# refresh-bio/fqsqueezer

Measured on AMD Instinct MI355X. Metric: Mbases/s compressed (DNA stream, SE sorted), higher is better.
Workload: dtype u64; 1 GPU; 1000000x150bp SE, G=7500000 (seed 2+rank), -om s -gs 8 -qm n -im n; workers_T=64, blocks=256, per_gpu=one independent file per GPU

## Files before the change

### fqsqueezer_amd/codec.py

```python
from __future__ import annotations

import ctypes as C
import os
from typing import List, Optional

import numpy as np

_PKG = os.path.dirname(os.path.abspath(__file__))
DEFAULT_LIB = os.path.join(_PKG, "libfqsx.so")

STAT_NAMES = ["gprobe", "gslot", "lprobe", "lslot", "gins", "gins_slot", "siv_words", "ctx_slots",
              "coded", "lins", "mail", "bases", "siv_saved", "dec_refetch"]


class FqsxError(RuntimeError):
    pass


_P, _INT, _U32, _U64, _HDR = C.c_void_p, C.c_int, C.c_uint32, C.c_uint64, C.c_char_p
_OUT, _U64S, _MS, _IN = C.POINTER(C.c_void_p), C.POINTER(C.c_uint64), C.POINTER(C.c_double), C.POINTER(C.c_char_p)
_ID_ENCODE = [_P, _P, _P, _U32, _INT, _OUT, _U64S]
_ID_DECODE = [_P, _IN, _P, _U32, _INT, _OUT, _OUT]

_ABI = {
    "fqsx_dna_create": (_INT, [_HDR, _INT, _OUT]),
    "fqsx_dna_create_on_partition": (_INT, [_HDR, _INT, _U32, _U32, _OUT]),
    "fqsx_dna_destroy": (None, [_P]),
    "fqsx_dna_use_chunked_tables": (_INT, [_P]),
    "fqsx_dna_encode_block": (_INT, [_P, _P, _P, _U32, _U32, _OUT, _U64S]),
    "fqsx_dna_encode_block_dev": (_INT, [_P, _P, _P, _P, _U32, _U32, _OUT, _U64S]),
    "fqsx_dna_decode_block": (_INT, [_P, _IN, _P, _P, _U32, _U32, _P]),
    "fqsx_dna_decode_block_dev": (_INT, [_P, _IN, _P, _P, _U32, _U32, _OUT]),
    "fqsx_dna_stats": (_INT, [_P, _U64S]),
    "fqsx_dna_capacity": (_INT, [_P, _U64S]),
    "fqsx_dna_set_profiling": (_INT, [_P, _INT]),
    "fqsx_dna_kernel_times": (_INT, [_P, _MS]),
    "fqsx_qual_create": (_INT, [_HDR, _INT, _OUT]),
    "fqsx_qual_destroy": (None, [_P]),
    "fqsx_qual_encode_block": (_INT, [_P, _P, _P, _U32, _OUT, _U64S]),
    "fqsx_qual_encode_block_dev": (_INT, [_P, _P, _P, _P, _U32, _OUT, _U64S]),
    "fqsx_qual_decode_block": (_INT, [_P, _IN, _P, _P, _U32, _P]),
    "fqsx_qual_decode_block_dev": (_INT, [_P, _IN, _P, _P, _U32, _OUT]),
    "fqsx_qual_contexts": (_INT, [_P, _P]),
    "fqsx_qual_set_profiling": (_INT, [_P, _INT]),
    "fqsx_qual_kernel_times": (_INT, [_P, _MS]),
# ... 637 lines not shown
```

### fqsqueezer_amd/csrc/fqsx_api.hip

```cpp
#include "fqsx_kernels.h"
#include "fqsx_qual.h"
#include "fqsx_qdec.h"
#include "../../include/fqsx.h"
#include "fqsx_vm.h"
#include "fqsx_rt.h"
#include <sys/resource.h>

#ifndef FQSX_EMU
#include <dlfcn.h>
#include <rccl/rccl.h>
#endif
#include <algorithm>
#include <cstdio>
#include <cstdlib>
#include <cstring>
#include <string>
#include <vector>

extern "C" const char *fqsx_last_error(void) { return g_err.c_str(); }
extern "C" const char *fqsx_version(void) {
#ifdef FQSX_EMU
  return "fqsx 0.1 (host emulation build - tests only)";
#else
  return "fqsx 0.1 (HIP gfx950)";
// ... 24 lines not shown
  }
  insert_phase_body(cfg, &sm, FQ_BLOCK / 3, FQ_BLOCK % 3);
  if (cfg.sys_scope) fq_release_system();
}
FQ_KERNEL64 void k_compact_generic(const u8 *out, u64 out_cap, const u64 *lens, u8 *dst) {
  const u32 tid = FQ_BLOCK;
  u64 off = 0;
  for (u32 t = 0; t < tid; ++t) off += lens[t];
  const u64 n = lens[tid] <= out_cap ? lens[tid] : 0;
  const u8 *src = out + (u64)tid * out_cap;
  for (u64 i = FQ_LANE; i < n; i += FQ_WAVE) dst[off + i] = src[i];
}
FQ_KERNEL64 void k_clear_local(DevCfg cfg, u64 nb_slots, u64 ns_slots) {
  if (phase_skip(cfg)) return;
  const u64 stride = (u64)FQ_NBLOCKS * FQ_WAVE, first = (u64)FQ_BLOCK * FQ_WAVE + FQ_LANE;
  for (u64 i = first; i < nb_slots; i += stride) cfg.l_b.slots[i] = 0;
  for (u64 i = first; i < ns_slots; i += stride) cfg.l_s.slots[i] = 0;
  for (u64 i = first; i < 2ull * cfg.T; i += stride) cfg.l_s.filled[i] = 0;
}
FQ_KERNEL64 void k_finish_block(DevCfg cfg, u64 *lens , u64 *end ) {
  if (FQ_LANE == 0) {
    if (FQ_BLOCK == 0) { end[2 * cfg.T] = cfg.err[0]; end[2 * cfg.T + 1] = cfg.err[1]; }
    if (cfg.err[1]) return;
    finish_block_body(cfg, FQ_BLOCK);
    lens[FQ_BLOCK] = cfg.ws[FQ_BLOCK].out_len;
    end[FQ_BLOCK] = cfg.ws[FQ_BLOCK].out_len;
    end[cfg.T + FQ_BLOCK] = cfg.ctx_filled[FQ_BLOCK];
  }
}
FQ_KERNEL64 void k_gather_stats(DevCfg cfg, u64 *out) {
  for (u32 i = FQ_LANE; i < 64; i += FQ_WAVE) {
    u64 s = 0;
    for (u32 t = 0; t < cfg.T; ++t) s += cfg.ws[t].stat[i];
    out[i] = s;
  }
}
FQ_DEV void part_split(const DevCfg &cfg, u32 &kind, u32 &blk) {
  kind = 0;
  blk = FQ_BLOCK;
  for (; kind < 2; ++kind) {
    const u32 g = cfg.T * cfg.mail[kind].n_tiles;
    if (blk < g) break;
    blk -= g;
  }
}
FQ_KERNEL64 void k_part_count(DevCfg cfg) {
  FQ_SHARED u32 hist[256];
  u32 kind, blk;
  if (phase_skip(cfg)) return;
  part_split(cfg, kind, blk);
  part_count_body(cfg, kind, blk, hist);
}
FQ_KERNEL64 void k_part_scan(DevCfg cfg) {
  if (phase_skip(cfg)) return;
  part_scan_body(cfg, FQ_BLOCK / cfg.T, FQ_BLOCK % cfg.T);
}
FQ_DEV void part_dstoff_leader(const DevCfg &cfg, u32 kind, u32 *demand , u32 seg1);
FQ_KERNEL64 void k_part_dstoff(DevCfg cfg, u32 *demand , u32 seg1) {
  if (cfg.err[0] || (cfg.err[1] && cfg.err[1] != seg1)) {
    if (FQ_BLOCK == 0 && FQ_LANE == 0) demand[2 * cfg.T] = cfg.err[0];
    return;
  }
  part_dstoff_leader(cfg, FQ_BLOCK, demand, seg1);
}
FQ_DEV void part_dstoff_leader(const DevCfg &cfg, u32 kind, u32 *demand, u32 seg1) {
  part_dstoff_body(cfg, kind);
  if (kind != MAIL_P)
// ... 1097 lines not shown
  if ((rc = dalloc(c, &p, T * sizeof(u32), true))) return rc;
  cfg.ctx_filled = (u32 *)p;
  {
    std::vector<u16> tpl(SM_OFF_BYTE, 0);
    auto fill = [&](u32 off, u32 entries, u32 stride, u32 n) {
      for (u32 e = 0; e < entries; ++e) {
        for (u32 i = 0; i < n; ++i) tpl[off + e * stride + i] = 1;
        tpl[off + e * stride + n] = (u16)n;
      }
    };
    fill(SM_OFF_FLAGS, 256, SM_FLAGS_N + 1, SM_FLAGS_N);
    fill(SM_OFF_NS, 32, SM_NS_N + 1, SM_NS_N);
    fill(SM_OFF_PSF, 65536, SM_PSF_N + 1, SM_PSF_N);
    fill(SM_OFF_PSNB, 65536, 6, cfg.ps_nobytes_n);
    fill(SM_OFF_NIB, 68, SM_NIB_N + 1, SM_NIB_N);
    tpl.resize(SM_TOTAL_U16, 0);
    fill(SM_OFF_MID, 1, SM_NIB_N + 1, SM_NIB_N);
    if ((rc = dalloc(c, &p, (u64)T * SM_TOTAL_U16 * sizeof(u16), false))) return rc;
    cfg.small = (u16 *)p;
    if ((rc = h2d(c, cfg.small, tpl.data(), tpl.size() * sizeof(u16)))) return rc;
    DEVCHK(dev_sync(c));
    for (u32 t = 1; t < T; ++t)
      if ((rc = d2d(c, cfg.small + (u64)t * SM_TOTAL_U16, cfg.small, tpl.size() * sizeof(u16)))) return rc;
    if ((rc = dalloc(c, &p, (u64)T * SM_LAZY_ENTRIES, true))) return rc;
    cfg.byte_init = (u8 *)p;
  }
  {
    std::vector<WState> ws(1);
    memset(ws.data(), 0, sizeof(WState));
    for (int g = 0; g < 4; ++g) {
      mt_seed(ws[0].mt[g], 5481);
      ws[0].mt_idx[g] = 624;
    }
    if ((rc = dalloc(c, &p, (u64)T * sizeof(WState), false))) return rc;
    cfg.ws = (WState *)p;
    for (u32 t = 0; t < T; ++t)
      if ((rc = h2d(c, cfg.ws + t, ws.data(), sizeof(WState)))) return rc;
    DEVCHK(dev_sync(c));
  }
  for (u32 k = 0; k < 3; ++k) {
    if ((rc = dalloc(c, &p, (u64)T * sizeof(u32), true))) return rc;
    cfg.mail[k].n = (u32 *)p;
    if ((rc = dalloc(c, &p, (u64)T * sizeof(u32), true))) return rc;
    cfg.mail[k].dst_tot = (u32 *)p;
    if ((rc = dalloc(c, &p, ((u64)T + 1) * sizeof(u32), true))) return rc;
    cfg.mail[k].dst_off = (u32 *)p;
    if ((rc = mail_alloc(c, k, FQSX_TILE))) return rc;
  }
  c->paired = cfg.mode >= 2;
  c->gpe_cap = c->lpe_cap = 0;
  if (c->paired) {
    c->gpe_cap = pow2_at_least(std::max<u64>(1024, (1ull << 20) / T));
    if (const char *e = getenv("FQSX_PTAB_INIT")) c->gpe_cap = pow2_at_least(std::max<u64>(64, strtoull(e, nullptr, 10)));
    if ((rc = ptab_alloc(c, cfg.g_pe, T, c->gpe_cap, true))) return rc;
    c->lpe_cap = 1024;
    if ((rc = ptab_alloc(c, cfg.l_pe, T, c->lpe_cap, true))) return rc;
    if ((rc = dalloc(c, &p, (u64)T * sizeof(u32), true))) return rc;
    cfg.pe_n = (u32 *)p;
    if ((rc = dalloc(c, &p, (3 * (u64)T + 1) * sizeof(u32), true))) return rc;
    cfg.pe_bkt_n = (u32 *)p;
    cfg.pe_bkt_cur = cfg.pe_bkt_n + 2 * T + 1;
  }
  {
    u8 ident[256];
    for (u32 i = 0; i < 256; ++i) ident[i] = (u8)i;
    if ((rc = dalloc(c, &p, 256, false))) return rc;
    c->d_vmap = (u8 *)p;
// ... 1952 lines not shown
```

### fqsqueezer_amd/csrc/fqsx_dev.h

```cpp
#pragma once
#include "fqsx_layout.h"
#include "fqsx_rc.h"

#define FQSX_RR 6u
#define FQSX_SW 4u
#define FQSX_NSC 3u
#define FQSX_SCR FQSX_NSC
#define FQSX_RQ 256u
struct SpecBuf {
  u32 h_read, h_i0, h_n;
  u32 h_epoch;
  u32 h_pub;
  u32 h_fix_lane, h_fix_end;
  u32 h_pq_lo[2];
  u32 h_np, h_nlp;
  u64 h_ns, h_nls;
  u64 sp_sdir[6][FQSX_SPEC];
  u64 sp_src[6][FQSX_SPEC];
  u8 sp_scur[6][FQSX_SPEC];
  u64 sp_key[10][FQSX_SPEC];
  u8 sp_kind[FQSX_SPEC];
  u64 sp_cq[FQSX_SPEC];
  u8 sp_lvz[FQSX_SPEC];
  u8 sp_flag[FQSX_SPEC];
// ... 144 lines not shown
  u32 pe_n;
  const u8 *din;
  u64 din_len, din_pos;
  RcDec dec;
  u32 la[3];
  u32 pq_lo[2];
  bool lqh;
  u32 lq_pub[2];
  u8 *rdp;
  SpecBuf *sb;
  bool scout;
  bool sc_abandoned;
  u32 sc_read;
  u32 sc_epoch;
  bool sc_poll;
  u32 nsc;
  bool sc_reqmode;
  const u8 *rq_p;
  u32 rq_size;
  bool rq_rev;
  u32 sc_taken;
  u32 sc_base;
  bool rq_early;
  bool rq_noscout;
  HeadRec *rec;
  u32 rec_idx;
  bool piped;
  u32 cq_tail, cq_head;
  bool rcq;
  u32 rq_tail;
  u64 c_r_sym;
  u64 st[ST_N];
  u64 tm[FQSX_TM_SLOTS];
  u32 err;
};
#define FQSX_TRACE_LAUNCHES 4096u
#define FQSX_TRACE_W 32u
#ifdef FQSX_TIMING
#define TM_STAMP(cfg, tid, launch, slot) do { if ((cfg).trace && (launch) < FQSX_TRACE_LAUNCHES && FQ_LANE == 0) (cfg).trace[((u64)(launch) * (cfg).T + (tid)) * FQSX_TRACE_W + (slot)] = fq_clock(); } while (0)
#define TM_TRACE_VAL(cfg, tid, launch, slot, v) do { if ((cfg).trace && (launch) < FQSX_TRACE_LAUNCHES && FQ_LANE == 0) (cfg).trace[((u64)(launch) * (cfg).T + (tid)) * FQSX_TRACE_W + (slot)] = (v); } while (0)
#else
#define TM_STAMP(cfg, tid, launch, slot) ((void)0)
#define TM_TRACE_VAL(cfg, tid, launch, slot, v) ((void)0)
#endif
#ifdef FQSX_TIMING
#define TM_BEGIN(v) u64 v = fq_clock()
#define TM_END(w, slot, v) (w).tm[slot] += fq_clock() - (v)
#define TM_COUNT(w, slot) (w).tm[slot] += 1
#if defined(FQSX_TIMING_PE)
#define TM_END_SP(w, slot, v) ((void)0)
#define TM_END_MD(w, slot, v) ((void)0)
#define TM_END_PE(w, slot, v) TM_END(w, slot, v)
#elif defined(FQSX_TIMING_MODELS)
#define TM_END_SP(w, slot, v) ((void)0)
#define TM_END_MD(w, slot, v) TM_END(w, slot, v)
#else
#define TM_END_SP(w, slot, v) TM_END(w, slot, v)
#define TM_END_MD(w, slot, v) ((void)0)
#endif
#ifndef TM_END_PE
#define TM_END_PE(w, slot, v) ((void)0)
#endif
#else
#define TM_BEGIN(v) ((void)0)
#define TM_END(w, slot, v) ((void)0)
#define TM_COUNT(w, slot) ((void)0)
// ... 2469 lines not shown
#endif
  TM_END(w, TM_CR_RC, t_rc);
  return L;
}
FQ_DEV u32 cq_process(Wk &w, u32 head, u32 avail) {
  u32 L = code_run(w, head, avail < 64 ? avail : 64);
  if (L == 0) {
    code_one(w, head);
    TM_COUNT(w, CN_P2);
    L = 1;
  }
  return L;
}
FQ_DEV void code_chunk(Wk &w, const u8 *p, u32 size, u32 i0, u32 j0, u32 m, bool reversed, u32 hist_start, bool &first) {
  if (m <= j0) return;
  TM_BEGIN(t_c2);
  WgShared *sm = w.sm;
  code_keys(w, p, size, i0, j0, m, reversed, hist_start);
  TM_END(w, TM_KEYS, t_c2);
  TM_BEGIN(t_cq);
  if (!cq_wait_space(w, m - j0)) return;
  for (u32 j = j0 + FQ_LANE; j < m; j += FQ_WAVE) {
    const u32 e = (w.cq_tail + (j - j0)) & (FQSX_CQ - 1);
    const u32 kind = w.sb->sp_kind[j];
    const u32 nk = kind == SK_LETTER ? 10u : 7u;
    for (u32 l = 0; l < nk; ++l) sm->cq_key[l][e] = w.sb->sp_key[l][j];
    sm->cq_kind[e] = (u8)(kind | (first && j == j0 ? SK_RESET : 0u));
    sm->cq_rsym[e] = w.sb->sp_rsym[j];
  }
  FQ_SYNC();
  first = false;
  cq_publish(w, m - j0);
  TM_END(w, TX_CHUNKQ, t_cq);
  if (!w.piped) {
    while (w.cq_head != w.cq_tail && !w.err) w.cq_head += cq_process(w, w.cq_head, w.cq_tail - w.cq_head);
    TM_END(w, TM_FAST, t_c2);
  }
}

#if FQ_WAVE > 1
FQ_DEV u32 grp_hash(u64 g) { return (u32)((g * 0x9E3779B97F4A7C15ull) >> 52); }
FQ_DEV void qm_set(u32 *bits, u64 g) {
  const u64 h = g * 0x9E3779B97F4A7C15ull;
  const u32 a = (u32)(h >> 51), b = (u32)(h >> 38) & 8191u;
  atomicOr(&bits[a >> 5], 1u << (a & 31));
  atomicOr(&bits[b >> 5], 1u << (b & 31));
}
FQ_DEV bool qm_test(const u32 *bits, u64 g) {
  const u64 h = g * 0x9E3779B97F4A7C15ull;
  const u32 a = (u32)(h >> 51), b = (u32)(h >> 38) & 8191u;
  return ((bits[a >> 5] >> (a & 31)) & (bits[b >> 5] >> (b & 31)) & 1u) != 0;
}
struct ConfMasks { u64 quiet, ncb, ncs; };
FQ_DEV ConfMasks conflict_masks(Wk &w, u32 n, bool want_quiet) {
  ConfMasks R;
  R.quiet = R.ncb = R.ncs = 0;
  SpecBuf *sb = w.sb;
  WgShared *sm = w.sm;
  const DevCfg *cfg = w.cfg;
  const u32 lane = FQ_LANE;
  FQ_SYNC();
  const u32 xfl = lane < n && sb->sp_flag[lane] == 3 ? sb->sx_flag[lane] : 0u;
  const bool cand = (xfl & SX_VALID) != 0, qcand = (xfl & (SX_VALID | SX_HITS)) == SX_VALID;
  const u64 A = wave_ballot(cand);
  if (popc64(A) < 4) return R;
  const u32 lo_b = w.pq_lo[0], hi_b = w.mn[MAIL_B], lo_s = w.pq_lo[1], hi_s = w.mn[MAIL_S];
// ... 639 lines not shown
      sm->cq_kind[e] = SK_RAW;
      sm->cq_rsym[e] = 5;
    }
    FQ_SYNC();
    cq_publish(w, n_raw);
  }
  if (!same) {
    mail_push(w, MAIL_P, rec->pmail[0]);
    mail_push(w, MAIL_P, rec->pmail[1]);
    w.pm.dir = rec->kdir[0]; w.pm.rc = rec->krc[0]; w.pm.cur = rec->kcur[0];
    w.sm_.dir = rec->kdir[1]; w.sm_.rc = rec->krc[1]; w.sm_.cur = rec->kcur[1];
    w.bm.dir = rec->kdir[2]; w.bm.rc = rec->krc[2]; w.bm.cur = rec->kcur[2];
    w.pm_u = w.pm; w.sm_u = w.sm_; w.bm_u = w.bm;
    w.cor_pos = 0;
    w.N_run = rec->n_run;
    w.rdp = sm->rd[idx % FQSX_HD];
    w.sc_read = idx;
    w.sc_abandoned = false;
    u32 hist[4] = {rec->hist[0], rec->hist[1], rec->hist[2], rec->hist[3]};
    TM_END(w, TM_READ_HEAD, t_head);
    suffix(w, p, size, false);
    add_s_letters(w, hist);
    w.st[ST_BASES] += size;
    if (w.sc_abandoned && has_next) scout_restart(w, idx + 1, w.cfg->pmer, w.s_let, SCQ_FROM_HEAD, false);
  }
  FQ_SYNC();
  lds_store_rel(&sm->hd_taken, idx + 1);
}

#include "fqsx_pe.h"
#include "fqsx_dec.h"


template <bool SPLIT>
FQ_DEV void coder_segment_body(const DevCfg &cfg, WgShared *sm, u32 tid, u32 seg, u32 launch = 0) {
  Wk w;
  w.cfg = &cfg;
  w.sm = sm;
  w.tid = tid;
  w.mode = 0;
  WState *ws = cfg.ws + tid;
  w.ws = ws;
  w.err = 0;
  w.piped = false;
  w.lqh = false;
  w.rec = nullptr;
  w.rdp = sm->rd[0];
  w.cq_head = w.cq_tail = 0;
  w.c_r_sym = 0;
  w.sb = &sm->sb[0];
  w.scout = false;
  for (u32 i = 0; i < ST_N; ++i) w.st[i] = 0;
  for (u32 i = 0; i < FQSX_TM_SLOTS; ++i) w.tm[i] = 0;
  w.rcq = SPLIT;
  w.rq_tail = 0;
  if (!SPLIT) {
    if (seg == 0) enc_open(w, 0, 0xff00000000000000ULL, 0, cfg);
    else enc_open(w, ws->rc_low, ws->rc_range, ws->out_len, cfg);
  }
  w.avg_code = ws->avg_code; w.avg_letters = ws->avg_letters;
  u32 head = 0, spins = 0;
  TM_BEGIN(t_all);
  for (;;) {
    const u32 done = lds_load_acq(&sm->cq_done);
    const u32 tail = lds_load_acq(&sm->cq_tail);
    if (tail != head) {
      TM_BEGIN(t_c);
      const u32 head0 = head;
      head += cq_process(w, head, tail - head);
      (void)head0;
      WHATIF(cfg, 2, (head >> 6) - (head0 >> 6));
      FQ_SYNC();
      lds_store_rel(&sm->cq_head, head);
      TM_END(w, TM_FAST, t_c);
      spins = 0;
    } else if (done) break;
    else {
      TM_BEGIN(t_idle);
      fq_sleep();
      if (spin_expired(spins)) { w.err = FQSX_ERR_PIPE; break; }
      TM_END(w, TM_CODER_IDLE, t_idle);
    }
  }
  TM_END(w, TM_P2, t_all);
  TM_STAMP(cfg, tid, launch, 3);
  if (SPLIT) {
    FQ_SYNC();
    lds_store_rel(&sm->rq_done, 1u);
  } else {
    enc_close(w);
    ws->rc_low = w.enc.low; ws->rc_range = w.enc.range; ws->out_len = w.enc.len;
  }
  ws->avg_code = w.avg_code; ws->avg_letters = w.avg_letters;
  if (FQ_LANE == 0) {
    for (u32 i = 0; i < ST_N; ++i) if (w.st[i]) atomic_add64(&ws->stat[i], w.st[i]);
#ifdef FQSX_TIMING
    for (u32 i = 0; i < FQSX_TM_SLOTS && i < 48; ++i) if (w.tm[i]) atomic_add64(&ws->stat[16 + i], w.tm[i]);
#endif
  }
  if (w.err) *cfg.err = w.err;
}

FQ_DEV void rc_segment_body(const DevCfg &cfg, WgShared *sm, u32 tid, u32 seg, u32 launch = 0) {
  Wk w;
  w.cfg = &cfg;
  w.sm = sm;
  w.tid = tid;
  w.mode = 0;
  WState *ws = cfg.ws + tid;
  w.ws = ws;
  w.err = 0;
  w.piped = false;
  w.lqh = false;
  w.rec = nullptr;
  w.rcq = false;
  w.scout = false;
  for (u32 i = 0; i < ST_N; ++i) w.st[i] = 0;
  for (u32 i = 0; i < FQSX_TM_SLOTS; ++i) w.tm[i] = 0;
  if (seg == 0) enc_open(w, 0, 0xff00000000000000ULL, 0, cfg);
  else enc_open(w, ws->rc_low, ws->rc_range, ws->out_len, cfg);
  u32 head = 0, spins = 0;
  for (;;) {
    const u32 done = lds_load_acq(&sm->rq_done);
    const u32 tail = lds_load_acq(&sm->rq_tail);
    if (tail != head) {
      TM_BEGIN(t_rc);
      const u32 n = tail - head < FQ_WAVE ? tail - head : FQ_WAVE;
// ... 424 lines not shown
  constexpr bool decode = DECODE, piped = PIPED;
  Wk w;
  w.cfg = &cfg;
  w.sm = sm;
  w.tid = tid;
  w.mode = (u32)MODE;
  WState *ws = cfg.ws + tid;
  w.ws = ws;
  w.err = 0;
  w.piped = piped;
  w.rcq = false;
  w.lqh = piped;
  w.rec = nullptr;
  w.rdp = sm->rd[0];
  constexpr bool heads = PIPED && MODE == 1;
  w.sb = &sm->sb[0];
  w.scout = PIPED && !(cfg.dbg & FQSX_DBG_SCOUTS_OFF);
  w.sc_reqmode = PIPED && MODE != 1;
  w.nsc = MODE >= 2 ? 2u : FQSX_NSC;
  w.rq_p = nullptr; w.rq_size = 0; w.rq_rev = false;
  w.sc_poll = false;
  w.sc_abandoned = false;
  w.sc_read = 0;
  w.sc_epoch = 0;
  w.sc_taken = 0;
  w.sc_base = 0;
  w.rq_early = false;
  w.rq_noscout = false;
  w.cq_head = w.cq_tail = 0;
  w.c_r_sym = 0;
  for (u32 i = 0; i < ST_N; ++i) w.st[i] = 0;
  for (u32 i = 0; i < FQSX_TM_SLOTS; ++i) w.tm[i] = 0;
  TM_BEGIN(t_total);
  TM_STAMP(cfg, tid, launch, 0);
  const u64 T = cfg.T;
  u64 first, last;
  worker_reads(tid, T, n_reads, first, last);
  if (seg == 0) {
    ws->cursor = (u32)first;
    if (!piped) {
      ws->rc_low = 0;
      ws->rc_range = 0xff00000000000000ULL;
      ws->out_len = 0;
    }
    ws->dec_pos = ~0ull;
  }
  constexpr bool paired = MODE >= 2;
  u64 stop;
  if (seg < S) {
    const u64 ns = segment_synchro(seg, S, first, last);
    if (!paired) stop = ns + 1;
    else {
      u64 i = ws->cursor;
      if (i < ns) i += (ns - i + 1) & ~1ull;
      stop = i + 2;
    }
  } else
    stop = last;
  if (stop > last) stop = last;
  FQ_SYNC();
  mt_copy((u64 *)&sm->mt[0][0], (const u64 *)&ws->mt[0][0]);
  for (u32 g = FQ_LANE; g < 4; g += FQ_WAVE) sm->mt_idx[g] = ws->mt_idx[g];
  w.mn[0] = w.mn[1] = w.mn[2] = 0;
  {
    u64 nu = cfg.siv_stats[0], nf = cfg.siv_stats[1];
    w.repm_gate = !((nf ? (double)nu / (double)nf : 0.0) < 7.0);
// ... 55 lines not shown
        prev_size = (u32)(q1 - q0);
      }
      compress_pair(w, cfg.bases + o0, (u32)(o1 - o0), cfg.bases + o1, (u32)(o2 - o1), prev, prev_size);
    }
  if (stop > cur) cur = stop;
  TM_STAMP(cfg, tid, launch, 6);
  lq_flush(w, MAIL_B);
  lq_flush(w, MAIL_S);

  if (piped) {
    FQ_SYNC();
    lds_store_rel(&sm->cq_done, 1u);
    lds_store_rel(&sm->lq_quit, 1u);
  }
  ws->cursor = (u32)cur;
  if (!piped) {
    if (decode) { ws->rc_low = w.dec.low; ws->rc_range = w.dec.range; }
    else {
      enc_close(w);
      ws->rc_low = w.enc.low; ws->rc_range = w.enc.range; ws->out_len = w.enc.len;
    }
    ws->avg_code = w.avg_code; ws->avg_letters = w.avg_letters;
  }
  for (u32 i = 0; i < 4; ++i) ws->s_letters[i] = w.s_let[i];
  ws->hidden_updates = w.hidden;
  TM_END(w, TM_TOTAL, t_total);
  TM_STAMP(cfg, tid, launch, 2);
  TM_TRACE_VAL(cfg, tid, launch, 8, w.tm[CN_SLOW]); TM_TRACE_VAL(cfg, tid, launch, 9, w.tm[CN_ROUGH]);
  TM_TRACE_VAL(cfg, tid, launch, 10, w.tm[CN_DIRTY]); TM_TRACE_VAL(cfg, tid, launch, 11, w.tm[CN_FAST]);
  TM_TRACE_VAL(cfg, tid, launch, 12, w.tm[TM_RRWAIT]); TM_TRACE_VAL(cfg, tid, launch, 13, w.tm[TM_SPEC]);
  TM_TRACE_VAL(cfg, tid, launch, 14, w.tm[CN_GENERIC]); TM_TRACE_VAL(cfg, tid, launch, 15, w.tm[TM_LQ]);
#ifdef FQSX_TIMING
  {
    const u32 xs[16] = {TM_SLOW, TM_SPRE, TM_ROUGH, TM_FINDC, TM_POST, TM_KEYS, TM_READ_HEAD, TM_CQWAIT, TX_QMM, TX_QRUN, TX_PROLOG, TX_CHUNKQ, TX_FLUSH, TM_TOTAL, TX_G_EARLY, TX_OWNSPEC};
    for (u32 x = 0; x < 16; ++x) TM_TRACE_VAL(cfg, tid, launch, 16 + x, w.tm[xs[x]]);
  }
#endif
  if (!piped) {
    for (u32 i = 0; i < ST_N; ++i) ws->stat[i] += w.st[i];
    for (u32 i = 0; i < FQSX_TM_SLOTS && i < 48; ++i) ws->stat[16 + i] += w.tm[i];
  } else if (FQ_LANE == 0) {
    for (u32 i = 0; i < ST_N; ++i) if (w.st[i]) atomic_add64(&ws->stat[i], w.st[i]);
#ifdef FQSX_TIMING
    for (u32 i = 0; i < FQSX_TM_SLOTS && i < 48; ++i) if (w.tm[i]) atomic_add64(&ws->stat[16 + i], w.tm[i]);
#endif
  }
  FQ_SYNC();
  mt_copy((u64 *)&ws->mt[0][0], (const u64 *)&sm->mt[0][0]);
  for (u32 g = FQ_LANE; g < 4; g += FQ_WAVE) ws->mt_idx[g] = sm->mt_idx[g];
  for (u32 k = 0; k < 3; ++k) cfg.mail[k].n[tid] = w.mn[k];
  if (paired) cfg.pe_n[tid] = w.pe_n;
  if (w.err) *cfg.err = w.err;
}

template <class SM>
FQ_DEV void insert_batch(const DevCfg &cfg, SM *sm, const KTab &t, u32 tid, const u64 *keys, u32 n, u32 rng, const Cinc &ci,
                         u64 &nslots, u32 &err) {
  insert_batch_k(cfg, sm, t, tid, FQ_LANE < n ? keys[FQ_LANE] : 0, n, rng, ci, nslots, err);
}
template <class SM>
FQ_DEV void insert_batch_k(const DevCfg &cfg, SM *sm, const KTab &t, u32 tid, u64 mykey, u32 n, u32 rng, const Cinc &ci,
                           u64 &nslots, u32 &err) {
  (void)cfg;
#ifdef FQSX_TIMING
  u64 ib_t[4] = {0, 0, 0, 0}, ib_rounds = 0;
#define IB_MARK(i) do { const u64 now_ = fq_clock(); ib_t[i] += now_ - ib_c; ib_c = now_; } while (0)
  u64 ib_c = fq_clock();
// ... 303 lines not shown
```

### fqsqueezer_amd/csrc/fqsx_layout.h

```cpp
#pragma once
#include "fqsx_plat.h"

#define FQSX_MAX_T 255
#define FQSX_SIV_BLK_LOG 14u
#define FQSX_SIV_BLK (1u << FQSX_SIV_BLK_LOG)
#define FQSX_NIL 0xffffffffu
#define FQSX_RD_LDS 3072u
#define FQSX_HD 3u
#define FQSX_SPEC 64u
#define FQSX_PQ 512u
#define FQSX_CQ 256u

struct KGeom {
  u32 k, shift;
  u64 mask, kernel_mask;
};

#define FQSX_BKT 4u
struct KTab {
  u64 *slots;
  u64 nb;
  u64 stride;
  u32 *filled;
  u32 k, cbits;
  u32 two, pad_;
};

struct CtxSlot {
  u64 key;
  u32 counter;
  u16 tag;
  u16 total;
  u16 st[5];
  u16 pad[3];
};

#define FQSX_TILE 2048u
struct Mail {
  u64 *list;
  u32 *n;
  u64 *sorted;
  u32 *tile_hist;
  u32 *dst_tot;
  u32 *dst_off;
// ... 28 lines not shown
#define SM_LAZY_ENTRIES (SM_BYTE_ENTRIES + SM_MPOS_ENTRIES)

struct WState {
  double avg_code, avg_letters;
  u64 ctx_flags, ctx_ps_flags;
  u64 s_letters[4];
  u64 pmer_prev_dir, pmer_prev_rc;
  u32 pmer_prev_cur;
  u32 cursor;
  u64 hidden_updates;
  u64 rc_low, rc_range;
  u64 out_len;
  u64 dec_buffer, dec_pos;
  u32 mt_idx[4];
  alignas(8) u32 mt[4][624];
  u64 stat[64];
};
enum { RNG_B = 0, RNG_S = 1, RNG_LB = 2, RNG_LS = 3 };
enum {
  ST_GPROBE = 0,
  ST_GSLOT,
  ST_LPROBE,
  ST_LSLOT,
  ST_GINS,
  ST_GINS_SLOT,
  ST_SIV_WORDS,
  ST_CTX,
  ST_CODED,
  ST_LINS,
  ST_MAIL,
  ST_BASES,
  ST_SIV_SAVED,
  ST_DEC_REFETCH,
  ST_N
};
enum { TM_TOTAL = 0, TM_SPEC, TM_FAST, TM_SLOW, TM_POST, TM_READ_HEAD, TM_LQ, TM_ROUGH, TM_REPM, TM_FINDC,
       CN_FAST, CN_SLOW, CN_CHUNK, CN_DIRTY, CN_ROUGH, CN_REPM,
       CN_EXT, CN_GENERIC, CN_LQFLUSH, TM_RRWAIT , TM_CQWAIT , CN_EARLY, CN_P2, TM_P2,
       TM_CODER_IDLE , TM_SCOUT_WAIT , TM_SPRE,
       TM_CR_S, TM_CR_MID, TM_CR_AVG, TM_CR_RC, TM_KEYS,
       TM_SC_SPEC , TM_SC_EARLY, TM_SC_ROUGH , TM_SC_IDLE , CN_SC_CHUNK, CN_SC_ABORT,
       TM_SP_ROLL , TM_SP_PROBE ,
       TM_N, TM_SP_HIT = 46 , TM_SP_MISS = 47 ,
       TX_QMM = 48 , TX_QRUN , TX_PROLOG ,
       TX_CHUNKQ , TX_FLUSH ,
       TX_G_EARLY , TX_OWNSPEC  };
#ifdef FQSX_TIMING
#define FQSX_TM_SLOTS 56
#else
#define FQSX_TM_SLOTS 1
#endif

struct DevCfg {
  u32 T, mode;
  u32 prefix, pmer, smer, bmer;
  KGeom gp, gs, gb;
  u32 pmer_mod_shift;
  u32 ps_nobytes_n;
  u64 T_magic;
  u32 T_pow2;
  u32 dbg;
  u64 *siv;
  u64 *siv_stats;
  u32 *siv_idx;
  KTab g_s, g_b;
  KTab l_s, l_b;
  CtxSlot *ctx;
  u64 ctx_cap_mask;
  u32 *ctx_filled;
  u16 *small;
  u8 *byte_init;
  WState *ws;
  Mail mail[3];
  PTab g_pe, l_pe;
  u64 *pe_list;
  u32 *pe_n;
  u32 pe_cap;
  u64 *pe_bkt;
  u32 *pe_bkt_n;
  u32 *pe_bkt_cur;
  const u8 *bases;
  const u64 *read_off;
  u8 *out;
  u64 out_cap;
  const u8 *din;
  const u64 *din_off;
  u8 *dout;
  u8 *dscratch;
  u64 dcap;
  u8 *pe_scr;
  u64 pe_scr_cap;
  u32 *err;
  u64 *trace;
  u32 shard_rank, shard_world;
  u32 tab_load_pct;
  u32 whatif;
  u32 sys_scope;
  u32 pe_part;
  u32 siv_part, pad_siv_;
  u64 *p_log;
  u32 *p_log_n;
  const u8 *vmap;
  u32 *shard_cnt;
};

enum {
  FQSX_DBG_SCOUTS_OFF = 1,
  FQSX_DBG_ABANDON = 2,
  FQSX_DBG_RESTART = 4,
  FQSX_DBG_INSERTER_STALL = 8,
};
enum {
  FQSX_ERR_OUT_OVERFLOW = 1,
  FQSX_ERR_GTAB_FULL = 2,
  FQSX_ERR_LTAB_FULL = 3,
  FQSX_ERR_CTX_FULL = 4,
  FQSX_ERR_MAIL_FULL = 5,
  FQSX_ERR_PE_FULL = 6,
  FQSX_ERR_PE_READ_TOO_LONG = 7,
  FQSX_ERR_DECODE = 8,
  FQSX_ERR_PIPE = 9,
};
```

### fqsqueezer_amd/csrc/fqsx_roles.h

```cpp
#pragma once
#include "fqsx_kernels.h"

template <int MODE> FQ_ROLE void role_resolve(FqArgsP ap) {
  const EncArgs *a = fq_args(ap);
  encode_segment_body<MODE, false, true>(a->cfg, fq_wg(), FQ_BLOCK, a->n_reads, a->S, a->seg, a->pad);
}
FQ_ROLE void role_models(FqArgsP ap) {
  const EncArgs *a = fq_args(ap);
  coder_segment_body<true>(a->cfg, fq_wg(), FQ_BLOCK, a->seg, a->pad);
}
FQ_ROLE void role_rc(FqArgsP ap) {
  const EncArgs *a = fq_args(ap);
  rc_segment_body(a->cfg, fq_wg(), FQ_BLOCK, a->seg, a->pad);
}
FQ_ROLE void role_inserter(FqArgsP ap) {
  const EncArgs *a = fq_args(ap);
  inserter_segment_body(a->cfg, fq_wg(), FQ_BLOCK, a->pad);
}
FQ_ROLE void role_head(FqArgsP ap) {
  const EncArgs *a = fq_args(ap);
  head_segment_body(a->cfg, fq_wg(), FQ_BLOCK, a->n_reads, a->S, a->seg, a->pad);
}
FQ_ROLE void role_scout(FqArgsP ap, u32 me_) {
  const EncArgs *a = fq_args(ap);
  scout_segment_body(a->cfg, fq_wg(), FQ_BLOCK, a->n_reads, a->S, a->seg, uniform32(me_), a->pad);
}
template <int NSC> FQ_ROLE void role_scout_req(FqArgsP ap, u32 me_) {
  const EncArgs *a = fq_args(ap);
  scout_request_body(a->cfg, fq_wg(), FQ_BLOCK, uniform32(me_), (u32)NSC, a->pad);
}

#ifndef FQSX_EMU
FQ_DEV bool worker_elsewhere(const EncArgs &a) {
  if (shard_mine(a.cfg, FQ_BLOCK)) return false;
  if (threadIdx.x == 0) {
    for (u32 k = 0; k < 3; ++k) a.cfg.mail[k].n[FQ_BLOCK] = 0;
    if (a.cfg.pe_n) a.cfg.pe_n[FQ_BLOCK] = 0;
  }
  return true;
}
FQ_DEV bool wg_handoff_init(const EncArgs &a, bool honour_posted) {
  WgShared *sm = fq_wg();
  if (threadIdx.x == 0) {
    sm->wg_stop = (a.cfg.err[0] | (honour_posted ? a.cfg.err[1] : 0u)) != 0 ? 1u : 0u;
    sm->cq_tail = 0; sm->cq_head = 0; sm->cq_done = 0;
    sm->lq_target[0] = sm->lq_target[1] = 0; sm->lq_done[0] = sm->lq_done[1] = 0; sm->lq_quit = 0;
    sm->hd_ready = 0; sm->hd_taken = 0; sm->hd_early = 0;
    sm->sc_taken = 0; sm->sc_req_seq = 0; sm->sc_dead = (a.cfg.dbg & FQSX_DBG_SCOUTS_OFF) ? 1u : 0u;
    for (u32 x = 0; x < FQSX_NSC; ++x) { sm->sc_hd_taken[x] = 0; sm->sc_ack[x] = 0; }
    for (u32 x = 1; x <= FQSX_SCR; ++x) sm->sb[x].h_pub = 0;
    sm->rq_tail = 0; sm->rq_head = 0; sm->rq_done = 0;
  }
  if (a.cfg.sys_scope && FQ_WAVE_ID == 0) fq_acquire_system();
  FQ_WG_BARRIER();
  return sm->wg_stop != 0;
}
#endif
```

Baseline: 110.3 Mbases/s.

## Carry unprocessed coding-queue entries across segment launches instead of draining

When the producer finishes a segment, the split coder role now spills its unconsumed coding-queue entries and range-coder symbol state to a per-worker global spill area, instead of draining the queue before the launch ends. The next segment launch restores those entries into LDS in wg_handoff_init and starts the queue head negative so the coder resumes on them. This is meant to remove the tail where the coder drains alone at each segment boundary, letting coding overlap with the next segment's producer. The cost is extra global memory traffic for the spill and restore, a larger WState allocation, and a debug lag mode plus timing counters.

```diff
diff --git a/fqsqueezer_amd/codec.py b/fqsqueezer_amd/codec.py
--- a/fqsqueezer_amd/codec.py
+++ b/fqsqueezer_amd/codec.py
@@ -10,7 +10,7 @@
 DEFAULT_LIB = os.path.join(_PKG, "libfqsx.so")
 
 STAT_NAMES = ["gprobe", "gslot", "lprobe", "lslot", "gins", "gins_slot", "siv_words", "ctx_slots",
-              "coded", "lins", "mail", "bases", "siv_saved", "dec_refetch"]
+              "coded", "lins", "mail", "bases", "siv_saved", "dec_refetch", "cq_carried"]
 
 
 class FqsxError(RuntimeError):
diff --git a/fqsqueezer_amd/csrc/fqsx_api.hip b/fqsqueezer_amd/csrc/fqsx_api.hip
--- a/fqsqueezer_amd/csrc/fqsx_api.hip
+++ b/fqsqueezer_amd/csrc/fqsx_api.hip
@@ -80,7 +80,7 @@
   for (u32 i = FQ_LANE; i < 64; i += FQ_WAVE) {
     u64 s = 0;
     for (u32 t = 0; t < cfg.T; ++t) s += cfg.ws[t].stat[i];
-    out[i] = s;
+    out[i] = i == ST_CQ_STATE ? 0 : s;
   }
 }
 FQ_DEV void part_split(const DevCfg &cfg, u32 &kind, u32 &blk) {
@@ -1244,7 +1244,8 @@
       mt_seed(ws[0].mt[g], 5481);
       ws[0].mt_idx[g] = 624;
     }
-    if ((rc = dalloc(c, &p, (u64)T * sizeof(WState), false))) return rc;
+    static_assert(sizeof(WState) % sizeof(u64) == 0, "the spill areas behind the WState array are u64 words");
+    if ((rc = dalloc(c, &p, (u64)T * (sizeof(WState) + FQSX_CQ_SPILL_U64 * sizeof(u64)), true))) return rc;
     cfg.ws = (WState *)p;
     for (u32 t = 0; t < T; ++t)
       if ((rc = h2d(c, cfg.ws + t, ws.data(), sizeof(WState)))) return rc;
diff --git a/fqsqueezer_amd/csrc/fqsx_dev.h b/fqsqueezer_amd/csrc/fqsx_dev.h
--- a/fqsqueezer_amd/csrc/fqsx_dev.h
+++ b/fqsqueezer_amd/csrc/fqsx_dev.h
@@ -200,6 +200,9 @@
   u64 c_r_sym;
   u64 st[ST_N];
   u64 tm[FQSX_TM_SLOTS];
+#ifdef FQSX_TIMING
+  u64 t_launch;
+#endif
   u32 err;
 };
 #define FQSX_TRACE_LAUNCHES 4096u
@@ -2735,6 +2738,9 @@
   first = false;
   cq_publish(w, m - j0);
   TM_END(w, TX_CHUNKQ, t_cq);
+#ifdef FQSX_TIMING
+  if (w.piped && !w.tm[TX_FIRSTCHUNK]) w.tm[TX_FIRSTCHUNK] = fq_clock() - w.t_launch;
+#endif
   if (!w.piped) {
     while (w.cq_head != w.cq_tail && !w.err) w.cq_head += cq_process(w, w.cq_head, w.cq_tail - w.cq_head);
     TM_END(w, TM_FAST, t_c2);
@@ -3440,8 +3446,26 @@
 #include "fqsx_dec.h"
 
 
+FQ_DEV u64 *cq_spill_area(const DevCfg &cfg, u32 tid) { return (u64 *)(cfg.ws + cfg.T) + (u64)tid * FQSX_CQ_SPILL_U64; }
+FQ_ROLE void cq_spill(u64 *sp, WState *ws, u32 head, u32 n, u32 r_sym) {
+  WgShared *sm = fq_wg();
+  u16 *kr = (u16 *)(sp + FQSX_CQ_SPILL_KR);
+  for (u32 i = FQ_LANE; i < n; i += FQ_WAVE) {
+    const u32 e = (head + i) & (FQSX_CQ - 1);
+    const u32 x = FQSX_CQ - n + i;
+    for (u32 l = 0; l < 10; ++l) sp[l * FQSX_CQ + x] = sm->cq_key[l][e];
+    kr[x] = (u16)(sm->cq_kind[e] | ((u32)sm->cq_rsym[e] << 8));
+  }
+  if (FQ_LANE == 0) {
+    ws->stat[ST_CQ_STATE] = (u64)n | ((u64)r_sym << 32);
+    if (n) atomic_add64(&ws->stat[ST_CQ_CARRIED], n);
+  }
+}
+static_assert(FQSX_HD_RAW <= FQSX_SPEC, "a producer never asks the coding queue for more than FQSX_SPEC entries at once (FQSX_DBG_CODER_LAG)");
 template <bool SPLIT>
-FQ_DEV void coder_segment_body(const DevCfg &cfg, WgShared *sm, u32 tid, u32 seg, u32 launch = 0) {
+FQ_DEV void coder_segment_body(const DevCfg &cfg, WgShared *sm, u32 tid, u32 seg, u32 launch = 0, bool carry_ = false) {
+  const bool carry = SPLIT && carry_;
+  const bool lag = SPLIT && (cfg.dbg & FQSX_DBG_CODER_LAG) != 0;
   Wk w;
   w.cfg = &cfg;
   w.sm = sm;
@@ -3455,7 +3479,7 @@
   w.rec = nullptr;
   w.rdp = sm->rd[0];
   w.cq_head = w.cq_tail = 0;
-  w.c_r_sym = 0;
+  w.c_r_sym = SPLIT && seg != 0 ? (u32)(ws->stat[ST_CQ_STATE] >> 32) : 0;
   w.sb = &sm->sb[0];
   w.scout = false;
   for (u32 i = 0; i < ST_N; ++i) w.st[i] = 0;
@@ -3467,17 +3491,22 @@
     else enc_open(w, ws->rc_low, ws->rc_range, ws->out_len, cfg);
   }
   w.avg_code = ws->avg_code; w.avg_letters = ws->avg_letters;
-  u32 head = 0, spins = 0;
+  u32 head = SPLIT ? uniform32(sm->cq_head) : 0u, spins = 0;
   TM_BEGIN(t_all);
   for (;;) {
     const u32 done = lds_load_acq(&sm->cq_done);
     const u32 tail = lds_load_acq(&sm->cq_tail);
-    if (tail != head) {
+    if (carry && done) {
+      if (tail - head > FQSX_CQ) w.err = FQSX_ERR_PIPE;
+      else cq_spill(cq_spill_area(cfg, tid), ws, head, tail - head, (u32)w.c_r_sym);
+      break;
+    }
+    if (tail != head && !(lag && !done && tail - head < FQSX_CQ - FQSX_SPEC)) {
       TM_BEGIN(t_c);
       const u32 head0 = head;
       head += cq_process(w, head, tail - head);
       (void)head0;
-      WHATIF(cfg, 2, (head >> 6) - (head0 >> 6));
+      WHATIF(cfg, 2, (u32)(((i32)head >> 6) - ((i32)head0 >> 6)));
       FQ_SYNC();
       lds_store_rel(&sm->cq_head, head);
       TM_END(w, TM_FAST, t_c);
@@ -3501,6 +3530,7 @@
   }
   ws->avg_code = w.avg_code; ws->avg_letters = w.avg_letters;
   if (FQ_LANE == 0) {
+    if (SPLIT && (!carry || w.err)) ws->stat[ST_CQ_STATE] = 0;
     for (u32 i = 0; i < ST_N; ++i) if (w.st[i]) atomic_add64(&ws->stat[i], w.st[i]);
 #ifdef FQSX_TIMING
     for (u32 i = 0; i < FQSX_TM_SLOTS && i < 48; ++i) if (w.tm[i]) atomic_add64(&ws->stat[16 + i], w.tm[i]);
@@ -3991,6 +4021,9 @@
   for (u32 i = 0; i < ST_N; ++i) w.st[i] = 0;
   for (u32 i = 0; i < FQSX_TM_SLOTS; ++i) w.tm[i] = 0;
   TM_BEGIN(t_total);
+#ifdef FQSX_TIMING
+  w.t_launch = t_total;
+#endif
   TM_STAMP(cfg, tid, launch, 0);
   const u64 T = cfg.T;
   u64 first, last;
@@ -4112,7 +4145,8 @@
   TM_TRACE_VAL(cfg, tid, launch, 14, w.tm[CN_GENERIC]); TM_TRACE_VAL(cfg, tid, launch, 15, w.tm[TM_LQ]);
 #ifdef FQSX_TIMING
   {
-    const u32 xs[16] = {TM_SLOW, TM_SPRE, TM_ROUGH, TM_FINDC, TM_POST, TM_KEYS, TM_READ_HEAD, TM_CQWAIT, TX_QMM, TX_QRUN, TX_PROLOG, TX_CHUNKQ, TX_FLUSH, TM_TOTAL, TX_G_EARLY, TX_OWNSPEC};
+    static_assert(TX_FIRSTCHUNK < FQSX_TM_SLOTS, "every TX_* timer needs a slot of Wk.tm");
+    const u32 xs[16] = {TM_SLOW, TM_SPRE, TM_ROUGH, TM_FINDC, TM_POST, TM_KEYS, TM_READ_HEAD, TM_CQWAIT, TX_QMM, TX_QRUN, TX_PROLOG, TX_CHUNKQ, TX_FLUSH, TM_TOTAL, TX_G_EARLY, TX_FIRSTCHUNK};
     for (u32 x = 0; x < 16; ++x) TM_TRACE_VAL(cfg, tid, launch, 16 + x, w.tm[xs[x]]);
   }
 #endif
diff --git a/fqsqueezer_amd/csrc/fqsx_layout.h b/fqsqueezer_amd/csrc/fqsx_layout.h
--- a/fqsqueezer_amd/csrc/fqsx_layout.h
+++ b/fqsqueezer_amd/csrc/fqsx_layout.h
@@ -10,6 +10,8 @@
 #define FQSX_SPEC 64u
 #define FQSX_PQ 512u
 #define FQSX_CQ 256u
+#define FQSX_CQ_SPILL_KR (10u * FQSX_CQ)
+#define FQSX_CQ_SPILL_U64 (FQSX_CQ_SPILL_KR + FQSX_CQ / 4u)
 
 struct KGeom {
   u32 k, shift;
@@ -104,8 +106,11 @@
   ST_BASES,
   ST_SIV_SAVED,
   ST_DEC_REFETCH,
-  ST_N
-};
+  ST_N,
+  ST_CQ_CARRIED = ST_N
+};
+enum { ST_CQ_STATE = 15 };
+static_assert(ST_CQ_CARRIED == 14 && ST_CQ_CARRIED < 16, "stat slot 14 (codec.py: STAT_NAMES); [16..63] are the section times");
 enum { TM_TOTAL = 0, TM_SPEC, TM_FAST, TM_SLOW, TM_POST, TM_READ_HEAD, TM_LQ, TM_ROUGH, TM_REPM, TM_FINDC,
        CN_FAST, CN_SLOW, CN_CHUNK, CN_DIRTY, CN_ROUGH, CN_REPM,
        CN_EXT, CN_GENERIC, CN_LQFLUSH, TM_RRWAIT , TM_CQWAIT , CN_EARLY, CN_P2, TM_P2,
@@ -116,7 +121,8 @@
        TM_N, TM_SP_HIT = 46 , TM_SP_MISS = 47 ,
        TX_QMM = 48 , TX_QRUN , TX_PROLOG ,
        TX_CHUNKQ , TX_FLUSH ,
-       TX_G_EARLY , TX_OWNSPEC  };
+       TX_G_EARLY , TX_OWNSPEC ,
+       TX_FIRSTCHUNK  };
 #ifdef FQSX_TIMING
 #define FQSX_TM_SLOTS 56
 #else
@@ -181,6 +187,7 @@
   FQSX_DBG_ABANDON = 2,
   FQSX_DBG_RESTART = 4,
   FQSX_DBG_INSERTER_STALL = 8,
+  FQSX_DBG_CODER_LAG = 16,
 };
 enum {
   FQSX_ERR_OUT_OVERFLOW = 1,
diff --git a/fqsqueezer_amd/csrc/fqsx_roles.h b/fqsqueezer_amd/csrc/fqsx_roles.h
--- a/fqsqueezer_amd/csrc/fqsx_roles.h
+++ b/fqsqueezer_amd/csrc/fqsx_roles.h
@@ -7,7 +7,7 @@
 }
 FQ_ROLE void role_models(FqArgsP ap) {
   const EncArgs *a = fq_args(ap);
-  coder_segment_body<true>(a->cfg, fq_wg(), FQ_BLOCK, a->seg, a->pad);
+  coder_segment_body<true>(a->cfg, fq_wg(), FQ_BLOCK, a->seg, a->pad, a->seg < a->S);
 }
 FQ_ROLE void role_rc(FqArgsP ap) {
   const EncArgs *a = fq_args(ap);
@@ -41,9 +41,22 @@
 }
 FQ_DEV bool wg_handoff_init(const EncArgs &a, bool honour_posted) {
   WgShared *sm = fq_wg();
+  static_assert(FQSX_CQ == 256u, "wg_handoff_init restores the coding queue with two threads of the 512 per entry");
+  if (a.seg != 0) {
+    const u64 *sp = cq_spill_area(a.cfg, FQ_BLOCK);
+    const u32 e = threadIdx.x & (FQSX_CQ - 1), l0 = (threadIdx.x >> 8) * 5u;
+    u64 k[5];
+    for (u32 x = 0; x < 5; ++x) k[x] = sp[(l0 + x) * FQSX_CQ + e];
+    if (threadIdx.x < FQSX_CQ) {
+      const u32 kr = ((const u16 *)(sp + FQSX_CQ_SPILL_KR))[e];
+      sm->cq_kind[e] = (u8)kr; sm->cq_rsym[e] = (u8)(kr >> 8);
+    }
+    for (u32 x = 0; x < 5; ++x) sm->cq_key[l0 + x][e] = k[x];
+  }
   if (threadIdx.x == 0) {
+    const u32 cq_n = a.seg != 0 ? (u32)a.cfg.ws[FQ_BLOCK].stat[ST_CQ_STATE] : 0u;
     sm->wg_stop = (a.cfg.err[0] | (honour_posted ? a.cfg.err[1] : 0u)) != 0 ? 1u : 0u;
-    sm->cq_tail = 0; sm->cq_head = 0; sm->cq_done = 0;
+    sm->cq_tail = 0; sm->cq_head = 0u - (cq_n < FQSX_CQ ? cq_n : FQSX_CQ); sm->cq_done = 0;
     sm->lq_target[0] = sm->lq_target[1] = 0; sm->lq_done[0] = sm->lq_done[1] = 0; sm->lq_quit = 0;
     sm->hd_ready = 0; sm->hd_taken = 0; sm->hd_early = 0;
     sm->sc_taken = 0; sm->sc_req_seq = 0; sm->sc_dead = (a.cfg.dbg & FQSX_DBG_SCOUTS_OFF) ? 1u : 0u;
```

After: 114.1 Mbases/s, median of 6. 3.4% higher.
